# eric-downes/tianshou_marl

Hardware: AMD Instinct MI355X
Metric: env-steps/sec (n_env x n_agent) incl. PPO update, simple_spread N=3 (higher is better)
Workload: dtype f32; 1 GPU; simple_spread_v3 N=3 shared PPO, num_envs=1024 per GPU, obs 18, A=5, T=25, MLP 64-64; minibatch=4096, repeat=1, dispatch=per_agent, parallelism=env-shard x1

## Files before the change

include/tsmarl.h:

```cpp
#ifndef TSMARL_H
#define TSMARL_H

#include <stdint.h>

#ifdef __cplusplus
extern "C" {
#endif

#define TSM_ABI_VERSION 4

enum {
    TSM_OK = 0,
    TSM_ERR_INVALID = 1,
    TSM_ERR_HIP = 2,
    TSM_ERR_MALFORMED_BUFFER = 3,
    TSM_ERR_UNSUPPORTED = 4
};
#define TSM_VALUE

TSM_VALUE int tsm_abi_version(void);
const char *tsm_last_error(void);
int tsm_device_info(int *n_cu, int *wave_size, int64_t *hbm_bytes, char *name_out);

int tsm_kernel_option_get(const char *name, int32_t *value_out);
// ... 202 lines not shown
    tsm_mpe_cfg env;
    uint64_t env_seed;
    uint64_t *episode_ctr;
    float *agent_pos, *agent_vel, *landmark_pos;
    int32_t *steps;
    int32_t auto_reset, n_steps;
    float *obs_cur_out;
    void *vrb_state;
    int64_t sub_size;
    uint8_t *done_store;
    float *obs_store, *obs_next_store, *rew_store, *logp_store, *vs_store, *vnext_store;
    int32_t *act_store;
    uint8_t *term_store, *trunc_store;
    int64_t *ptr_out;
    double *ep_rew_out;
    int64_t *ep_len_out, *ep_idx_out;
    int64_t *ep_rec;
    int32_t max_ep, _pad2;
    uint64_t offset_inc;
    uint32_t *done_ctr;
} tsm_rollout_desc;

int tsm_rollout_spread(const tsm_rollout_desc *desc_host, void *stream);
int tsm_rollout_spread_actor(const tsm_rollout_desc *desc, void *stream);

typedef struct {
    int32_t n_env, n_adv, n_good, n_obst, max_cycles, _pad;
    double dt, damping, contact_force, contact_margin;
    double adv_size, good_size, obst_size;
    double adv_accel, good_accel, adv_speed, good_speed;
} tsm_mpe_tag_cfg;
TSM_VALUE int tsm_mpe_tag_obs_dim(const tsm_mpe_tag_cfg *cfg_host);
int tsm_mpe_tag_reset(const tsm_mpe_tag_cfg *cfg_host, uint64_t seed, uint64_t *episode_ctr,
                      const int64_t *env_ids, int64_t n_ids, float *agent_pos, float *agent_vel,
                      float *landmark_pos, int32_t *steps, float *obs_out, void *stream);
int tsm_mpe_tag_step(const tsm_mpe_tag_cfg *cfg_host, uint64_t seed, uint64_t *episode_ctr, const int32_t *act,
                     float *agent_pos, float *agent_vel, float *landmark_pos, int32_t *steps, float *obs_next_out,
                     float *obs_cur_out, float *rew_out, uint8_t *terminated_out, uint8_t *truncated_out,
                     uint8_t *done_env_out, int auto_reset, uint64_t *rng_tick, uint64_t rng_tick_inc, void *stream);
int tsm_u64_add(uint64_t *counter, uint64_t inc, void *stream);

typedef struct {
    const float *params[2];
    uint64_t policy_seed[2], offset[2];
    int32_t mode[2];
    int32_t obs_dim, hidden, n_act;
// ... 391 lines not shown
```

tianshou_marl_amd/algorithm/ppo.py:

```python
from __future__ import annotations

import os
import time
from typing import Literal

import numpy as np
import torch
from torch import nn

from .. import ops
from ..data.batch import Batch, split_bounds
from ..data.buffer import DeviceVectorReplayBuffer
from ..data.stats import (A2CTrainingStats, LazyDict, MapTrainingStats, ResultRing, lazy_training_stats, pinned_slot,
                          training_stats_from_steps)
from ..utils.net import DeviceRunningMeanStd, DiscreteActorCritic
from ..utils.tensor import to_tensor


class PPO(nn.Module):
    def __new__(cls, *args, **kw):
        if cls is PPO and kw.get("policy") is not None and kw.get("net") is None:
            from ..utils.net import MLPActorCritic, net_from_reference_modules

            if isinstance(net_from_reference_modules(kw["policy"], kw.get("critic"), kw.get("device", "cuda")), MLPActorCritic):
# ... 29 lines not shown
            lr, betas, adam_eps, weight_decay = kw_o["lr"], kw_o["betas"], kw_o["adam_eps"], kw_o["weight_decay"]
            sched_factory = getattr(optim, "lr_scheduler_factory", None)
        self._ctor = dict(lr=lr, betas=betas, adam_eps=adam_eps, weight_decay=weight_decay, eps_clip=eps_clip,
                          dual_clip=dual_clip, value_clip=value_clip, advantage_normalization=advantage_normalization,
                          recompute_advantage=recompute_advantage, vf_coef=vf_coef, ent_coef=ent_coef,
                          max_grad_norm=max_grad_norm, gae_lambda=gae_lambda, max_batchsize=max_batchsize, gamma=gamma,
                          return_scaling=return_scaling, deterministic_eval=deterministic_eval, dispatch=dispatch,
                          shuffle=shuffle, seed=seed, use_graph=use_graph, async_stats=async_stats)
        self._sched_factory = sched_factory
        self.net = net
        from ..env.spaces import Box, Discrete

        self.action_space = Discrete(net.n_act)
        self.observation_space = Box(-np.inf, np.inf, (net.obs_dim,))
        self._lr_dev = torch.tensor([float(lr)], dtype=torch.float64, device=net.flat.device)
        self._lr = float(lr)
        self.lr_schedulers: list = []
        if sched_factory is not None:
            self.lr_schedulers.append(sched_factory.create_scheduler(self))
        self.betas, self.adam_eps, self.weight_decay = betas, adam_eps, weight_decay
        self.eps_clip, self.dual_clip, self.value_clip = eps_clip, dual_clip, value_clip
        self.advantage_normalization, self.recompute_adv = advantage_normalization, recompute_advantage
        self.pack_rows = True
        self.vf_coef, self.ent_coef, self.max_grad_norm = vf_coef, ent_coef, max_grad_norm
        self.gae_lambda, self.gamma, self.max_batchsize = gae_lambda, gamma, max_batchsize
        self.return_scaling, self.ret_rms, self._eps = return_scaling, DeviceRunningMeanStd(net.flat.device), 1e-8
        self.deterministic_eval = deterministic_eval
        self.reuse_rollout_outputs = True
        self.is_within_training_step = False
        self.dispatch, self.shuffle = dispatch, shuffle
        self.use_graph = use_graph
        self.async_stats = async_stats
        self.seed = int(seed)
        dev = net.flat.device
        self.exp_avg = torch.zeros_like(net.flat.data)
        self.exp_avg_sq = torch.zeros_like(net.flat.data)
        self.opt_step = 0
        self._adam_work = torch.zeros(ops.call("tsm_adam_work_elems", net.flat.numel()), dtype=torch.float32, device=dev)
        self._sample_ctr = 0
        self._perm_ctr = torch.zeros(1, dtype=torch.int64, device=dev)
        self._cfg = ops.make_ppo_cfg(eps_clip, dual_clip, value_clip, advantage_normalization, vf_coef, ent_coef)
        self._ws: dict = {}
        self._grad_sync = None
        self.graph_collectives = os.environ.get("TSM_GRAPH_COLLECTIVES", "1") != "0"
        self.param_version = 0

# ... 26 lines not shown

    def forward(self, batch: Batch, state=None, **kwargs) -> Batch:
        obs = batch.obs
        if isinstance(obs, Batch) and "observations" in obs:
            from ..data.buffer import _obs_array

            obs = _obs_array(obs)
        elif isinstance(obs, Batch) and "obs" in obs:
            obs = obs.obs
        obs_t = torch.as_tensor(np.asarray(obs) if not isinstance(obs, torch.Tensor) else obs).to(self.device, torch.float32)
        lead = obs_t.shape[:-1]
        res = self.act_device(obs_t)
        return Batch(logits=res["logits"].reshape(*lead, -1), act=res["act"].reshape(lead).to(torch.int64),
                     state=None, policy=Batch(logp=res["logp"].reshape(lead), v_s=res["value"].reshape(lead)))

    def map_action(self, act):
        return act

    def map_action_inverse(self, act):
        return act

    def add_exploration_noise(self, act, batch):
        return act

    def _valid_rows(self, buffer: DeviceVectorReplayBuffer):
        lengths = buffer.index.lengths
        lens_h = lengths.cpu().numpy()
        S, B = buffer.sub_size, buffer.buffer_num
        uniform = bool((lens_h == lens_h[0]).all())
        ins_h = buffer.index.insertion_idx.cpu().numpy()
        start_h = (ins_h - lens_h) % S
        if uniform and (start_h == 0).all():
            T = int(lens_h[0])
            return T, None, None, None
        k = np.arange(S)[None, :]
        slot = (start_h[:, None] + k) % S
        valid = k < lens_h[:, None]
        rows = (slot * B + np.arange(B)[:, None])[valid]
        dev = self.device
        return S, torch.as_tensor(rows).to(dev), torch.as_tensor(start_h.astype(np.int32)).to(dev), \
            torch.as_tensor(lens_h.astype(np.int32)).to(dev)

    def _preprocess_batch(self, buffer: DeviceVectorReplayBuffer) -> dict:
        T, rows, env_start, env_len = self._valid_rows(buffer)
        B, N, D = buffer.buffer_num, buffer.n_agent, buffer.obs_dim
        L = B * N
# ... 309 lines not shown
            if self.advantage_normalization and not self.recompute_adv:
                seg = torch.arange(len(groups) * repeat, dtype=torch.int64, device=dev).view(-1, 1) * n_g
                w["mb_start_all"] = torch.cat([(seg + w["mb_start"][:-1].view(1, -1)).reshape(-1),
                                               torch.tensor([len(groups) * repeat * n_g], dtype=torch.int64, device=dev)])

            def preprocess(recompute: bool = False):
                if stored and not recompute:
                    if self.recompute_adv:
                        w["v_s"].copy_(buffer.vs_store[:T].reshape(T, L))
                        w["v_next"].copy_(buffer.vnext_store[:T].reshape(T, L))
                else:
                    img = self.net.image if recompute else None
                    ops.policy_forward(P, obs, A, H, mode="none" if recompute else "given", act=act,
                                       image=img,
                                       out=dict(value=w["v_s"].view(-1), logp=None if recompute else w["logp"],
                                                logits=None))
                    if no_next:
                        self._next_values_by_index(buffer, w["v_s"], T, None, out=w["v_next"])
                    else:
                        ops.policy_forward(P, obs_next, A, H, mode="none", image=img,
                                           out=dict(value=w["v_next"].view(-1), logits=None))
                self._gae(w["v_s"], w["v_next"], rew, term, trunc, N, out=(w["ret"], w["adv"]))

            def body():
                if self.shuffle == "device":
                    ops.random_permutations(n_g, len(groups) * repeat, self.seed ^ 0x5DEECE66D, counter_dev=w["step_dev"],
                                            scale=N if per_agent else 1, group_size=repeat,
                                            offset_mul=1 if per_agent else 0, out=w["perm"])
                preprocess()
                if "mb_start_all" in w and w["packed"] is not None:
                    ops.ppo_pack_minibatches(w["packed"], w["adv"], w["mb_start_all"], w["perm"].view(-1), obs, act, w["logp"],
                                             w["ret"].view(-1), w["v_s"].view(-1) if self.value_clip else None,
                                             out=w["stats"].view(-1, 2))
                    yield from self._global_adv_stats_steps(w["stats"].view(-1, 2), w["mb_start_all"])
                elif "mb_start_all" in w:
                    ops.ppo_adv_stats(w["adv"], w["mb_start_all"], perm=w["perm"].view(-1), out=w["stats"].view(-1, 2),
                                      max_rows=w["max_rows"])
                    yield from self._global_adv_stats_steps(w["stats"].view(-1, 2), w["mb_start_all"])
                pb = dict(obs=obs, act=act, logp_old=w["logp"], adv=w["adv"].view(-1), ret=w["ret"].view(-1),
                          v_s=w["v_s"].view(-1))
                k = 0
                for gi in range(len(groups)):
                    for r in range(repeat):
                        if self.recompute_adv and r > 0:
                            preprocess(recompute=True)
                        perm = w["perm"][gi, r]
                        if self.advantage_normalization and "mb_start_all" not in w:
                            ops.ppo_adv_stats(w["adv"], w["mb_start"], perm=perm, out=w["stats"][gi, r],
                                              max_rows=w["max_rows"])
                            yield from self._global_adv_stats_steps(w["stats"][gi, r], w["mb_start"])
                        for j, (s, e) in enumerate(bounds):
                            yield from self._grad_step_steps(
                                pb, perm[s:e], w["stats"][gi, r, j] if self.advantage_normalization else None, w["step_dev"],
                                plan=w, partial=w["partial"][k], image=self.net.image if k > 0 else None,
                                packed=None if w["packed"] is None else w["packed"]["rows"](k))
                            k += 1

            ops.capture_steps(w, body, self._sum_over_ranks, capture=self._capture_graph,
                              segmented=self._grad_sync is not None and not self.graph_collectives)
            if self.shuffle == "numpy":
                w["ref_ids"] = self._ref_ids(T, B, N, groups)
            self._ws[key] = g = w
        self._refill_host_perms(g)
        self._refill_step_dev(g)
        ops.replay_steps(g, self._sum_over_ranks)
        self._account_steps(g)
        slot = ResultRing.of(g, lambda: pinned_slot(*g["scal"].shape)).take(
            "expire" if self.async_stats else "resolve", "training stats were not read within 4 update() calls (async_stats=True)")
        ops.ppo_finalize_many(g["partial"], g["nb_max"] * 4, g["nb_dev"], g["M_dev"], self._cfg, slot["h"])
        sync = self._grad_sync
        if sync is not None:
            sync.post_check()
        slot["event"].record()

        out = lazy_training_stats(slot, sync, N if per_agent else None)
        if not self.async_stats:
            out.resolve()
        return out

    def update(self, buffer: DeviceVectorReplayBuffer, batch_size: int | None, repeat: int):
        if not self.is_within_training_step:
            raise RuntimeError(
                "update() was called outside of a training step as signalled by `is_within_training_step=False`; "
                "wrap the call in `policy_within_training_step(policy)` (tianshou/utils/torch_utils.py:31-46)")
        t0 = time.time()
        out = self._update(buffer, batch_size, repeat, t0)
        for sched in self.lr_schedulers:
            sched.step()
        out.train_time = time.time() - t0
# ... 331 lines not shown
```

tianshou_marl_amd/csrc/perm.hip:

```cpp
#include "common.h"
#include "philox.h"

namespace {

__device__ __forceinline__ uint32_t mix32(uint32_t x) {
    x ^= x >> 16; x *= 0x7feb352dU;
    x ^= x >> 15; x *= 0x846ca68bU;
    x ^= x >> 16;
    return x;
}

__device__ __forceinline__ void perm_point(int64_t n, int hb, uint64_t seed, uint64_t ctr, int64_t i, int p, int64_t scale,
                                           int32_t group_size, int64_t offset_mul, int64_t *__restrict__ out) {
    uint32_t k[4];
    tsm_philox4(seed, ctr + (uint64_t)p, k);
    const uint32_t mask = (1u << hb) - 1u;
    uint32_t x = (uint32_t)i;
    do {
        uint32_t l = x >> hb, r = x & mask;
#pragma unroll
        for (int round = 0; round < 6; ++round) {
            const uint32_t f = mix32(r + k[round & 3] + 0x9E3779B9u * (uint32_t)(round + 1)) & mask;
            const uint32_t t = l ^ f;
            l = r;
            r = t;
        }
        x = (l << hb) | r;
    } while ((int64_t)x >= n);
    out[(int64_t)p * n + i] = (int64_t)x * scale + (int64_t)(p / group_size) * offset_mul;
}

__global__ __launch_bounds__(256) void perm_kernel(int64_t n, int hb, uint64_t seed, uint64_t counter,
                                                    const uint64_t *__restrict__ counter_dev, int64_t scale,
                                                    int32_t group_size, int64_t offset_mul, int64_t *__restrict__ out) {
    const int64_t i = (int64_t)blockIdx.x * 256 + threadIdx.x;
    if (i >= n) return;
    perm_point(n, hb, seed, counter + (counter_dev ? *counter_dev : 0), i, blockIdx.y, scale, group_size, offset_mul, out);
}

__global__ __launch_bounds__(256) void perm_advance_kernel(int64_t n, int hb, uint64_t seed, uint64_t *counter_dev, uint64_t inc,
                                                            uint32_t *done_ctr, int64_t scale, int32_t group_size,
                                                            int64_t offset_mul, int64_t *__restrict__ out) {
    const uint64_t ctr = __hip_atomic_load(counter_dev, __ATOMIC_RELAXED, __HIP_MEMORY_SCOPE_AGENT);
    const int64_t i = (int64_t)blockIdx.x * 256 + threadIdx.x;
    if (i < n) perm_point(n, hb, seed, ctr, i, blockIdx.y, scale, group_size, offset_mul, out);
    __syncthreads();
    if (threadIdx.x == 0 && atomicAdd(done_ctr, 1u) == gridDim.x * gridDim.y - 1) {
        __hip_atomic_store(counter_dev, ctr + inc, __ATOMIC_RELAXED, __HIP_MEMORY_SCOPE_AGENT);
        *done_ctr = 0u;
    }
}

}

TSM_EXPORT int tsm_random_permutations(int64_t n, int32_t n_perm, uint64_t seed, uint64_t counter,
                                       const uint64_t *counter_dev, int64_t scale, int32_t group_size,
                                       int64_t offset_mul, int64_t *out, void *stream) {
    TSM_REQUIRE(n >= 0 && n < ((int64_t)1 << 30), "tsm_random_permutations: n=%lld out of range [0, 2^30)", (long long)n);
    TSM_REQUIRE(n_perm >= 0 && n_perm <= 65535, "tsm_random_permutations: n_perm out of range");
    TSM_REQUIRE(group_size >= 1, "tsm_random_permutations: group_size must be >= 1");
    if (n == 0 || n_perm == 0) return TSM_OK;
    TSM_REQUIRE(out, "tsm_random_permutations: null output");
    int bits = 0;
    while (((int64_t)1 << bits) < n) ++bits;
    const int hb = bits < 2 ? 1 : (bits + 1) / 2;
    hipLaunchKernelGGL(perm_kernel, dim3((unsigned)ceil_div(n, 256), (unsigned)n_perm), dim3(256), 0, tsm_stream(stream),
                       n, hb, seed, counter, counter_dev, scale, group_size, offset_mul, out);
    TSM_LAUNCH_CHECK();
    return TSM_OK;
}

TSM_EXPORT int tsm_random_permutations_advance(int64_t n, int32_t n_perm, uint64_t seed, uint64_t *counter_dev, uint64_t counter_inc,
                                               uint32_t *done_ctr, int64_t scale, int32_t group_size, int64_t offset_mul,
                                               int64_t *out, void *stream) {
    TSM_REQUIRE(n >= 1 && n < ((int64_t)1 << 30), "tsm_random_permutations_advance: n=%lld out of range [1, 2^30)", (long long)n);
    TSM_REQUIRE(n_perm >= 1 && n_perm <= 65535, "tsm_random_permutations_advance: n_perm out of range");
    TSM_REQUIRE(group_size >= 1, "tsm_random_permutations_advance: group_size must be >= 1");
    TSM_REQUIRE(out && counter_dev && done_ctr, "tsm_random_permutations_advance: null pointer");
    int bits = 0;
    while (((int64_t)1 << bits) < n) ++bits;
    const int hb = bits < 2 ? 1 : (bits + 1) / 2;
    hipLaunchKernelGGL(perm_advance_kernel, dim3((unsigned)ceil_div(n, 256), (unsigned)n_perm), dim3(256), 0, tsm_stream(stream),
                       n, hb, seed, counter_dev, counter_inc, done_ctr, scale, group_size, offset_mul, out);
    TSM_LAUNCH_CHECK();
    return TSM_OK;
}
```

tianshou_marl_amd/csrc/rollout.hip:

```cpp
#include "common.h"
#include "mlp_tile.h"
#include "mpe_dev.h"
#include "philox.h"
#include "rollout_dev.h"
#include "rollout_fwd.h"
#include "wave_mlp.h"

int tsm_mpe_check_cfg(const tsm_mpe_cfg *h, MpeCfg *c);
extern long long *g_tsm_stamps;

namespace {

struct RolloutArgs {
    const float *P, *img;
    Dims d;
    uint64_t pol_seed, offset;
    const uint64_t *offset_dev;
    int mode;
    MpeCfg c;
    uint64_t env_seed;
    uint64_t *episode_ctr;
    float *apos, *avel, *lpos;
    int32_t *steps;
    int auto_reset;
    float *obs_cur_out;
    RolloutBufArgs b;
    long long *stamps;
};


#define XSTAMP(k) do { if (a.stamps && blockIdx.x == 0 && threadIdx.x == 0 && t < 4) a.stamps[900 + t * 8 + (k)] = (long long)wall_clock64(); } while (0)
#define STAMP(k) do { if (a.stamps && blockIdx.x == 0 && threadIdx.x == 0 && t < 4) a.stamps[t * 8 + (k)] = (long long)wall_clock64(); } while (0)

struct RtLay {
    int XN0, AP, AV, LP, REW, LOGP, VAL, MIN, ACT, STEPS, DONE, ROW, EP, CX, CY, CV, U, ANY, total;
    __host__ __device__ RtLay(int fwd_total, int ld1) {
        int o = fwd_total;
        XN0 = o; o += R * ld1;
        AP = o; o += R * 2;
        AV = o; o += R * 2;
        LP = o; o += R * 2;
        REW = o; o += R;
        LOGP = o; o += R;
        VAL = o; o += R;
        MIN = o; o += R;
        ACT = o; o += R;
        STEPS = o; o += R;
        DONE = o; o += 2 * R;
        o = (o + 1) & ~1;
        ROW = o; o += 2 * 2 * R;
        EP = o; o += 2 * R;
        o = (o + 3) & ~3;
        CX = o; o += R * 8;
        CY = o; o += R * 8;
        CV = o; o += R * 8;
        U = o; o += 2 * R;
        ANY = o; o += 2;
        o += 3 * R + 12;
        total = o;
    }
};

template <int H, int NT2, int DS = 0, int NS = 0>
__global__ __launch_bounds__(NT2) void rollout_kernel(RolloutArgs a) {
    extern __shared__ __attribute__((aligned(16))) float lds[];
    const Dims d = DS ? dims_const(DS, 5) : a.d;
    MpeCfg c_ = a.c;
    if (NS) { c_.N = NS; c_.obs_dim = DS; }
    const MpeCfg c = c_;
    const Lay<H> ly(d, false);
    const int N = c.N, D = d.D, st = 2 * N;
    const int EPB = R / N;
    const int e0 = blockIdx.x * EPB;
    const int n_here = min(EPB, c.n_env - e0);
    const int rows_here = n_here * N;
    const int64_t B = c.n_env;
    const RtLay tl(ly.total, d.ld1);
    float *XN0 = lds + tl.XN0, *s_ap = lds + tl.AP, *s_av = lds + tl.AV, *s_lp = lds + tl.LP, *s_rew = lds + tl.REW,
          *s_logp = lds + tl.LOGP, *s_val = lds + tl.VAL, *s_m = lds + tl.MIN, *s_cx = lds + tl.CX, *s_cy = lds + tl.CY, *s_u = lds + tl.U;
    int *s_act = reinterpret_cast<int *>(lds + tl.ACT), *s_steps = reinterpret_cast<int *>(lds + tl.STEPS),
        *s_done = reinterpret_cast<int *>(lds + tl.DONE), *s_cv = reinterpret_cast<int *>(lds + tl.CV),
        *s_any = reinterpret_cast<int *>(lds + tl.ANY);
    int64_t *s_row = reinterpret_cast<int64_t *>(lds + tl.ROW);
    uint64_t *s_ep = reinterpret_cast<uint64_t *>(lds + tl.EP);

    if (a.stamps && threadIdx.x == 0 && blockIdx.x < 256) a.stamps[64 + 2 * blockIdx.x] = (long long)wall_clock64();
    const bool main_t = threadIdx.x < NT;
    if (main_t) {
// ... 255 lines not shown
                    const int rr = i / D, k = i - rr * D, ee = rr / N;
                    if (s_done[g + ee])
                        XN[rr * d.ld1 + k] =
                            mpe_obs_elem(c, s_ap + ee * st, s_av + ee * st, s_lp + ee * st, rr - ee * N, k);
                }
                __syncthreads();
            }
        }
        { const int tmp = xcur; xcur = xnxt; xnxt = tmp; }
        STAMP(6);
    }
    __syncthreads();
    if (a.stamps && threadIdx.x == 0 && blockIdx.x < 256) a.stamps[65 + 2 * blockIdx.x] = (long long)wall_clock64();
    for (int i = threadIdx.x; i < n_here * st; i += NT2) {
        a.apos[(int64_t)e0 * st + i] = s_ap[i];
        a.avel[(int64_t)e0 * st + i] = s_av[i];
        a.lpos[(int64_t)e0 * st + i] = s_lp[i];
    }
    if (env_lane) {
        a.steps[be] = s_steps[bel];
        vl.store(vs, a.b.ep_rec, be);
    }
    if (ret_lane) epr.store(vs, N, e0 + rq);
    rollout_advance_counter(a.b.done_ctr, a.b.offset_dev_rw, a.b.offset_inc, threadIdx.x == 0);
}

struct Rw64Lay {
    static constexpr int kLdc = 68;
    int AP, AV, LP, LG, H2C, VAL, CX, CY, CV, MIN, REW, LOGP, ACT, STEPS, DONE, ROW, EP, size;
    __host__ __device__ Rw64Lay() {
        int q = 0;
        AP = q; q += 2 * R;
        AV = q; q += 2 * R;
        LP = q; q += 2 * R;
        LG = q; q += R * 16;
        H2C = q; q += R * kLdc;
        VAL = q; q += R;
        CX = q; q += R * 8;
        CY = q; q += R * 8;
        CV = q; q += R * 8;
        MIN = q; q += R;
        REW = q; q += R;
        LOGP = q; q += R;
        ACT = q; q += R;
        STEPS = q; q += R;
        DONE = q; q += R;
        ROW = q; q += 2 * R;
// ... 248 lines not shown
        a.apos[(int64_t)e0 * st + lane] = s_ap[lane];
        a.avel[(int64_t)e0 * st + lane] = s_av[lane];
        a.lpos[(int64_t)e0 * st + lane] = s_lp[lane];
    }
    if (env_lane) {
        a.steps[be] = s_steps[bel];
        vl.store(vs, a.b.ep_rec, be);
        epr.store(vs, N, be);
    }
    rollout_advance_counter(a.b.done_ctr, a.b.offset_dev_rw, a.b.offset_inc, tid == 0);
}

__global__ void u64_add_kernel(uint64_t *p, uint64_t inc) { *p += inc; }

}

TSM_EXPORT int tsm_u64_add(uint64_t *counter, uint64_t inc, void *stream) {
    TSM_REQUIRE(counter, "tsm_u64_add: null pointer");
    hipLaunchKernelGGL(u64_add_kernel, dim3(1), dim3(1), 0, tsm_stream(stream), counter, inc);
    TSM_LAUNCH_CHECK();
    return TSM_OK;
}

TSM_EXPORT int tsm_rollout_spread(const tsm_rollout_desc *desc_host, void *stream) {
    TSM_REQUIRE(desc_host, "tsm_rollout_spread: null descriptor");
    const tsm_rollout_desc &h = *desc_host;
    RolloutArgs a;
    if (int rc = make_dims(h.obs_dim, h.hidden, h.n_act, &a.d)) return rc;
    if (int rc = tsm_mpe_check_cfg(&h.env, &a.c)) return rc;
    TSM_REQUIRE(a.c.obs_dim == h.obs_dim, "tsm_rollout_spread: obs_dim %d != 6 * n_agent", h.obs_dim);
    TSM_REQUIRE(h.n_act == 5, "tsm_rollout_spread: simple_spread has 5 discrete actions");
    TSM_REQUIRE(a.c.N <= R, "tsm_rollout_spread: n_agent exceeds the row tile");
    TSM_REQUIRE(h.n_steps >= 1 && h.sub_size >= 1, "tsm_rollout_spread: bad n_steps / sub_size");
    TSM_REQUIRE(h.mode == 1 || h.mode == 2, "tsm_rollout_spread: mode must be 1 (sample) or 2 (argmax)");
    TSM_REQUIRE((h.params || h.param_image) && h.episode_ctr && h.agent_pos && h.agent_vel && h.landmark_pos && h.steps,
                "tsm_rollout_spread: null pointer");
    if (int rc = rollout_buf_args(h, "tsm_rollout_spread", &a.b)) return rc;
    a.P = h.params; a.img = h.param_image;
    a.pol_seed = h.policy_seed; a.offset = h.offset; a.offset_dev = h.offset_dev; a.mode = h.mode;
    a.env_seed = h.env_seed; a.episode_ctr = h.episode_ctr;
    a.apos = h.agent_pos; a.avel = h.agent_vel; a.lpos = h.landmark_pos; a.steps = h.steps;
    a.auto_reset = h.auto_reset; a.obs_cur_out = h.obs_cur_out;
    a.stamps = g_tsm_stamps;
    const Lay<64> ly(a.d, false);
    {
        const int form = tsm_opt(TSM_OPT_ROLLOUT_FORM);
        const int64_t total_waves = ceil_div(a.c.n_env, R / a.c.N);
        if (a.d.nJ <= 3 && (form == 2 || (form == 0 && total_waves > 256))) {
            int n_waves = 1;
            while (n_waves < 4 && ceil_div(total_waves, n_waves) > 256) n_waves *= 2;
// ... 20 lines not shown
            } else
            switch (a.d.nJ) {
                case 1: LAUNCHW(1); break;
                case 2: LAUNCHW(2); break;
                default: LAUNCHW(3); break;
            }
#undef LAUNCHW
            TSM_LAUNCH_CHECK();
            return TSM_OK;
        }
    }
    const size_t shmem = (size_t)RtLay(ly.total, a.d.ld1).total * sizeof(float);
    static bool attr_set = false;
    if (!attr_set) {
        TSM_HIP(tsm_allow_max_lds(reinterpret_cast<const void *>(rollout_kernel<64, NT>)));
        TSM_HIP(tsm_allow_max_lds(reinterpret_cast<const void *>(rollout_kernel<64, 2 * NT>)));
        TSM_HIP(tsm_allow_max_lds(reinterpret_cast<const void *>(rollout_kernel<64, 2 * NT, 18, 3>)));
        attr_set = true;
    }
    const int EPB = R / a.c.N;
    const unsigned n_wg = (unsigned)ceil_div(a.c.n_env, EPB);
    const bool eight = n_wg <= 256 || shmem > 80 * 1024;
    const bool c18 = a.d.D == 18 && a.d.A == 5 && a.c.N == 3 && !tsm_opt(TSM_OPT_GENERIC);
    if (eight && c18) hipLaunchKernelGGL((rollout_kernel<64, 2 * NT, 18, 3>), dim3(n_wg), dim3(2 * NT), shmem, tsm_stream(stream), a);
    else if (eight) hipLaunchKernelGGL((rollout_kernel<64, 2 * NT>), dim3(n_wg), dim3(2 * NT), shmem, tsm_stream(stream), a);
    else hipLaunchKernelGGL((rollout_kernel<64, NT>), dim3(n_wg), dim3(NT), shmem, tsm_stream(stream), a);
    TSM_LAUNCH_CHECK();
    return TSM_OK;
}
```

tianshou_marl_amd/csrc/rollout_dev.h:

```cpp
#pragma once
#include "common.h"
#include "vrb_dev.h"

struct RolloutBufArgs {
    void *vrb_state;
    int64_t S;
    uint8_t *done_store;
    float *obs_store, *obs_next_store, *rew_store, *logp_store, *vs_store, *vnext_store;
    int32_t *act_store;
    uint8_t *term_store, *trunc_store;
    int64_t *ptr_out, *ep_len_out, *ep_idx_out;
    double *ep_rew_out;
    int n_steps;
    int64_t *ep_rec;
    int max_ep;
    uint64_t offset_inc;
    uint64_t *offset_dev_rw;
    uint32_t *done_ctr;
};

template <class Desc>
int rollout_buf_args(const Desc &h, const char *entry, RolloutBufArgs *b) {
    TSM_REQUIRE(h.vrb_state && h.done_store && h.obs_store && h.act_store && h.rew_store && h.term_store && h.trunc_store &&
                    h.ptr_out && h.ep_rew_out && h.ep_len_out && h.ep_idx_out,
// ... 25 lines not shown
        for (int k = 0; k < MAXN; ++k) if (k < N) acc[k] = vs.ep_return[be * N + k];
    }
    __device__ __forceinline__ void fold(double *ep_rew_out, int64_t *ep_rec, int max_ep, int N, int64_t B, int64_t be, int64_t o, bool tr,
                                         bool rec, int &n_fin, const float *rew) {
        double *rec_rew = rec ? reinterpret_cast<double *>(ep_rec + B + (int64_t)B * max_ep) +
                                    ((int64_t)be * max_ep + n_fin) * N : nullptr;
#pragma unroll
        for (int k = 0; k < MAXN; ++k) {
            if (k < N) {
                const double ac = acc[k] + (double)rew[k];
                ep_rew_out[o * N + k] = tr ? ac : 0.0;
                if (rec) rec_rew[k] = ac;
                acc[k] = tr ? 0.0 : ac;
            }
        }
        n_fin += tr ? 1 : 0;
    }
    __device__ __forceinline__ void store(const VrbState &vs, int N, int64_t be) const {
#pragma unroll
        for (int k = 0; k < MAXN; ++k) if (k < N) vs.ep_return[be * N + k] = acc[k];
    }
};

__device__ __forceinline__ void rollout_advance_counter(uint32_t *done_ctr, uint64_t *offset_dev_rw, uint64_t offset_inc, bool first) {
    if (done_ctr && first) {
        if (atomicAdd(done_ctr, 1u) == gridDim.x - 1) {
            *offset_dev_rw += offset_inc;
            *done_ctr = 0u;
        }
    }
}
```

tianshou_marl_amd/data/collector.py:

```python
from __future__ import annotations

import time
import warnings
from copy import copy
from typing import Any, Callable

import numpy as np
import torch

from .. import ops
from .batch import Batch
from .buffer import DeviceVectorReplayBuffer
from .stats import CollectStats, ResultRing


_EXPIRED = ("these CollectStats were not read within 4 collect() calls and their pinned staging buffer was recycled "
            "(Collector(async_stats=True)); read them earlier or use async_stats=False")


class LazyCollectStats(CollectStats):

    _LAZY = ("returns", "lens", "n_collected_episodes", "returns_stat", "lens_stat")

    def __init__(self, collector: "Collector", slot: dict, steps: int) -> None:
# ... 38 lines not shown
                self.__dict__[k] = getattr(full, k)
            self._col.collect_episode += self.__dict__["n_collected_episodes"]
            object.__setattr__(self, "_done", True)
            if slot["pending"] is self:
                slot["pending"] = None
        return self

    def __getattribute__(self, name):
        if name in LazyCollectStats._LAZY and not object.__getattribute__(self, "_done"):
            object.__getattribute__(self, "resolve")()
        return object.__getattribute__(self, name)


class Collector:
    def __init__(self, policy, env, buffer: DeviceVectorReplayBuffer | None = None, exploration_noise: bool = False,
                 on_episode_done_hook: Callable | None = None, on_step_hook: Callable | None = None,
                 raise_on_nan_in_buffer: bool = False, collect_stats_class: type = CollectStats, use_graph: bool = True,
                 fused_rollout: bool = True, async_stats: bool = False) -> None:
        self.use_graph = use_graph
        self.async_stats = async_stats
        self.collect_stats_class = collect_stats_class
        self.fused_rollout = fused_rollout
        self.stage_episode_record = False
        self.policy = getattr(policy, "policy", policy)
        self.env = env
        self.env_num = len(env)
        if buffer is None:
            raise ValueError("a DeviceVectorReplayBuffer is required (the buffer lives in HBM)")
        if hasattr(buffer, "bind") and not buffer.allocated and hasattr(env, "n_agent") and hasattr(env, "obs_dim"):
            buffer.bind(env.n_agent, env.obs_dim)
        if buffer.buffer_num < self.env_num:
            raise ValueError(f"Buffer has only {buffer.buffer_num} sub-buffers for {self.env_num} envs")
        self.buffer = buffer
        self.exploration_noise = exploration_noise
        self.on_episode_done_hook, self.on_step_hook = on_episode_done_hook, on_step_hook
        self.raise_on_nan_in_buffer = raise_on_nan_in_buffer
        self.collect_step = self.collect_episode = 0
        self.collect_time = 0.0
        self._pre_obs = None
        self._pre_info = None
        self._pred_std: list = []
        self._device_path = hasattr(env, "step_device") and hasattr(self.policy, "act_device")
        self._ws: dict = {}
        if self._device_path:
            from ..utils.host import warn_if_oversubscribed

# ... 231 lines not shown
    def _rollout_fused(self, n_iter: int, ws: dict, deterministic: bool, rec_host=None) -> None:
        import ctypes as C

        from .._abi import call, ptr, stream_ptr, tsm_rollout_desc

        env, buf, pol = self.env, self.buffer, self._single_policy()
        if hasattr(env, "_tag_cfg"):
            return self._rollout_fused_tag(n_iter, ws, rec_host)
        actor_only = self._can_fuse_actor()
        actor = self._actor_of(pol) if actor_only else None
        entry = "tsm_rollout_spread_actor" if actor_only else "tsm_rollout_spread"

        def mark():
            if actor_only:
                buf.policy_outputs_version = None
                buf.behaviour_outputs_version = None
                buf.column_outputs = None
                buf.mark_logp_outputs(getattr(pol, "param_version", None))
            else:
                buf.mark_policy_outputs(getattr(pol, "param_version", -1))
                buf.mark_column_outputs([(id(pol), getattr(pol, "param_version", None))] * buf.n_agent)
            buf.note_uniform_rows(n_iter)

        img = getattr(getattr(pol, "net", None), "image", None)
        flat = actor.flat.data if actor_only else pol.net.flat.data
        ctr0 = int(getattr(pol, "_sample_ctr", 0))
        dkey = ("desc", n_iter, deterministic, env._pp, pol.seed, ctr0, env._seed, int(env.auto_reset), buf.storage_key(),
                flat.data_ptr(), 0 if img is None else img.data_ptr(), env.agent_pos.data_ptr())
        if dkey in self._ws:
            d = self._ws[dkey]
            d.ep_rec = rec_host.data_ptr() if rec_host is not None else None
            call(entry, C.byref(d), stream_ptr())
            mark()
            return
        d = tsm_rollout_desc()
        self._ws[dkey] = d
        d.params, d.param_image = ptr(flat), None
        d.obs_dim, d.hidden, d.n_act, d.mode = env.obs_dim, (128 if actor_only else pol.net.hidden), env.n_act, 2 if deterministic else 1
        d.policy_seed, d.offset, d.offset_dev = pol.seed & (2**64 - 1), ctr0, ptr(env.rng_tick)
        d.env, d.env_seed, d.episode_ctr = env._cfg, env._seed & (2**64 - 1), ptr(env.episode_ctr)
        d.agent_pos, d.agent_vel, d.landmark_pos = ptr(env.agent_pos), ptr(env.agent_vel), ptr(env.landmark_pos)
        d.steps, d.auto_reset, d.n_steps = ptr(env.steps), int(env.auto_reset), n_iter
        d.obs_cur_out = ptr(env.obs_cur)
        d.vrb_state, d.sub_size, d.done_store = ptr(buf.index.state), buf.sub_size, ptr(buf.done_store)
        d.obs_store, d.obs_next_store, d.rew_store = ptr(buf.obs_store), ptr(buf.obs_next_store), ptr(buf.rew_store)
        d.logp_store, d.vs_store, d.vnext_store = ptr(buf.logp_store), ptr(buf.vs_store), ptr(buf.vnext_store)
        d.act_store, d.term_store, d.trunc_store = ptr(buf.act_store), ptr(buf.term_store), ptr(buf.trunc_store)
        d.ptr_out, d.ep_rew_out = ptr(ws["ptr"]), ptr(ws["ep_rew"])
        d.ep_len_out, d.ep_idx_out = ptr(ws["ep_len"]), ptr(ws["ep_idx"])
        if rec_host is not None:
            d.ep_rec, d.max_ep = rec_host.data_ptr(), ws["max_ep"]
        if "done_ctr" not in ws:
            ws["done_ctr"] = torch.zeros(1, dtype=torch.int32, device=buf.device)
        d.offset_inc, d.done_ctr = n_iter * self.env_num * buf.n_agent, ptr(ws["done_ctr"])
        call(entry, C.byref(d), stream_ptr())
        mark()

    def _rollout_fused_tag(self, n_iter: int, ws: dict, rec_host=None) -> None:
        import ctypes as C

        from .._abi import call, ptr, stream_ptr, tsm_rollout_tag_desc

        env, buf = self.env, self.buffer
        teams = self._tag_teams()
        modes = tuple(2 if (getattr(p, "deterministic_eval", False) and not getattr(p, "is_within_training_step", False))
                      else 1 for p in teams)
        dkey = ("tag_desc", n_iter, modes, env._pp, tuple(p.seed for p in teams), tuple(p._sample_ctr for p in teams),
                env._seed, int(env.auto_reset), buf.storage_key(), tuple(p.net.flat.data_ptr() for p in teams),
                env.agent_pos.data_ptr())
        d = self._ws.get(dkey)
        if d is None:
            d = tsm_rollout_tag_desc()
            self._ws[dkey] = d
            for k, p in enumerate(teams):
                d.params[k], d.policy_seed[k], d.offset[k] = ptr(p.net.flat.data), p.seed & (2**64 - 1), p._sample_ctr
                d.mode[k] = modes[k]
            d.obs_dim, d.hidden, d.n_act, d.offset_dev = env.obs_dim, 64, env.n_act, ptr(env.rng_tick)
            d.env_major_counter = int(teams[0] is teams[1])
# ... 241 lines not shown
```

Measured before the change: 171.6 million env-steps/s.

## Generate PPO minibatch permutations in idle workgroups of the rollout kernel

Adds extra workgroups to the fused spread rollout launch. When the grid is smaller than the CU count, these fill the next PPO update's device permutation buffer on otherwise idle CUs. The PPO update then replays a separately captured graph that skips the permutation kernel, saving one launch and its serial time. In exchange it adds handshake state between collector and policy, a second captured graph, and a completion counter that must now count only rollout tiles. It also depends on the step counter being unchanged between rollout and update.

```diff
diff --git a/include/tsmarl.h b/include/tsmarl.h
--- a/include/tsmarl.h
+++ b/include/tsmarl.h
@@ -248,6 +248,10 @@
 } tsm_rollout_desc;
 
 int tsm_rollout_spread(const tsm_rollout_desc *desc_host, void *stream);
+int tsm_rollout_spread_prep(const tsm_rollout_desc *desc_host, int64_t perm_n, int32_t n_perm, uint64_t perm_seed,
+                            const uint64_t *perm_counter_dev, int64_t perm_scale, int32_t perm_group_size,
+                            int64_t perm_offset_mul, int64_t *perm_out, int32_t n_cu, int32_t *taken_out, void *stream);
+int tsm_rollout_prep_extra(int64_t tiles, int32_t n_cu, int64_t perm_n, int32_t n_perm, int32_t *extra_out);
 int tsm_rollout_spread_actor(const tsm_rollout_desc *desc, void *stream);
 
 typedef struct {
diff --git a/tianshou_marl_amd/algorithm/ppo.py b/tianshou_marl_amd/algorithm/ppo.py
--- a/tianshou_marl_amd/algorithm/ppo.py
+++ b/tianshou_marl_amd/algorithm/ppo.py
@@ -75,6 +75,10 @@
         self.eps_clip, self.dual_clip, self.value_clip = eps_clip, dual_clip, value_clip
         self.advantage_normalization, self.recompute_adv = advantage_normalization, recompute_advantage
         self.pack_rows = True
+        self.rollout_prep = True
+        self._prep_offer = None
+        self._prep_gen = 0
+        self._prep_filled = None
         self.vf_coef, self.ent_coef, self.max_grad_norm = vf_coef, ent_coef, max_grad_norm
         self.gae_lambda, self.gamma, self.max_batchsize = gae_lambda, gamma, max_batchsize
         self.return_scaling, self.ret_rms, self._eps = return_scaling, DeviceRunningMeanStd(net.flat.device), 1e-8
@@ -147,6 +151,19 @@
 
     def add_exploration_noise(self, act, batch):
         return act
+
+    def rollout_prep_request(self, buffer: DeviceVectorReplayBuffer) -> dict | None:
+        self._prep_filled = None
+        if not (self.rollout_prep and self.is_within_training_step and self._prep_offer is not None):
+            return None
+        key, g = self._prep_offer
+        if self._ws.get(key) is not g or key[1] != buffer.storage_key() or g.get("step_host") != self.opt_step:
+            return None
+        self._prep_gen += 1
+        return dict(g["perm_request"], gen=self._prep_gen, key=key)
+
+    def rollout_prep_done(self, req: dict, taken: bool) -> None:
+        self._prep_filled = (req["gen"], req["key"], self.opt_step) if taken else None
 
     def _valid_rows(self, buffer: DeviceVectorReplayBuffer):
         lengths = buffer.index.lengths
@@ -502,8 +519,10 @@
                                            out=dict(value=w["v_next"].view(-1), logits=None))
                 self._gae(w["v_s"], w["v_next"], rew, term, trunc, N, out=(w["ret"], w["adv"]))
 
+            skip_perm = [False]
+
             def body():
-                if self.shuffle == "device":
+                if self.shuffle == "device" and not skip_perm[0]:
                     ops.random_permutations(n_g, len(groups) * repeat, self.seed ^ 0x5DEECE66D, counter_dev=w["step_dev"],
                                             scale=N if per_agent else 1, group_size=repeat,
                                             offset_mul=1 if per_agent else 0, out=w["perm"])
@@ -540,11 +559,35 @@
                               segmented=self._grad_sync is not None and not self.graph_collectives)
             if self.shuffle == "numpy":
                 w["ref_ids"] = self._ref_ids(T, B, N, groups)
+            if (self.shuffle == "device" and self._grad_sync is None and not self.recompute_adv
+                    and self.advantage_normalization and w["packed"] is not None):
+                w["perm_request"] = dict(out=w["perm"], n=n_g, n_perm=len(groups) * repeat, seed=self.seed ^ 0x5DEECE66D,
+                                         counter_dev=w["step_dev"], scale=N if per_agent else 1, group_size=repeat,
+                                         offset_mul=1 if per_agent else 0)
+
+                def capture_prepared():
+                    w2: dict = {}
+                    skip_perm[0] = True
+                    try:
+                        ops.capture_steps(w2, body, self._sum_over_ranks, capture=self._capture_graph)
+                    finally:
+                        skip_perm[0] = False
+                    w["graph_prep"] = w2["graph"]
+
+                w["capture_prepared"] = capture_prepared
             self._ws[key] = g = w
         self._refill_host_perms(g)
-        self._refill_step_dev(g)
-        ops.replay_steps(g, self._sum_over_ranks)
+        filled, self._prep_filled = self._prep_filled, None
+        if (self.rollout_prep and "perm_request" in g and g.get("step_host") == self.opt_step
+                and filled == (self._prep_gen, key, self.opt_step)):
+            if g.get("graph_prep") is None:
+                g["capture_prepared"]()
+            g["graph_prep"].replay()
+        else:
+            self._refill_step_dev(g)
+            ops.replay_steps(g, self._sum_over_ranks)
         self._account_steps(g)
+        self._prep_offer = (key, g) if self.rollout_prep and "perm_request" in g else None
         slot = ResultRing.of(g, lambda: pinned_slot(*g["scal"].shape)).take(
             "expire" if self.async_stats else "resolve", "training stats were not read within 4 update() calls (async_stats=True)")
         ops.ppo_finalize_many(g["partial"], g["nb_max"] * 4, g["nb_dev"], g["M_dev"], self._cfg, slot["h"])
diff --git a/tianshou_marl_amd/csrc/perm.hip b/tianshou_marl_amd/csrc/perm.hip
--- a/tianshou_marl_amd/csrc/perm.hip
+++ b/tianshou_marl_amd/csrc/perm.hip
@@ -1,34 +1,8 @@
 #include "common.h"
+#include "perm_dev.h"
 #include "philox.h"
 
 namespace {
-
-__device__ __forceinline__ uint32_t mix32(uint32_t x) {
-    x ^= x >> 16; x *= 0x7feb352dU;
-    x ^= x >> 15; x *= 0x846ca68bU;
-    x ^= x >> 16;
-    return x;
-}
-
-__device__ __forceinline__ void perm_point(int64_t n, int hb, uint64_t seed, uint64_t ctr, int64_t i, int p, int64_t scale,
-                                           int32_t group_size, int64_t offset_mul, int64_t *__restrict__ out) {
-    uint32_t k[4];
-    tsm_philox4(seed, ctr + (uint64_t)p, k);
-    const uint32_t mask = (1u << hb) - 1u;
-    uint32_t x = (uint32_t)i;
-    do {
-        uint32_t l = x >> hb, r = x & mask;
-#pragma unroll
-        for (int round = 0; round < 6; ++round) {
-            const uint32_t f = mix32(r + k[round & 3] + 0x9E3779B9u * (uint32_t)(round + 1)) & mask;
-            const uint32_t t = l ^ f;
-            l = r;
-            r = t;
-        }
-        x = (l << hb) | r;
-    } while ((int64_t)x >= n);
-    out[(int64_t)p * n + i] = (int64_t)x * scale + (int64_t)(p / group_size) * offset_mul;
-}
 
 __global__ __launch_bounds__(256) void perm_kernel(int64_t n, int hb, uint64_t seed, uint64_t counter,
                                                     const uint64_t *__restrict__ counter_dev, int64_t scale,
@@ -61,9 +35,7 @@
     TSM_REQUIRE(group_size >= 1, "tsm_random_permutations: group_size must be >= 1");
     if (n == 0 || n_perm == 0) return TSM_OK;
     TSM_REQUIRE(out, "tsm_random_permutations: null output");
-    int bits = 0;
-    while (((int64_t)1 << bits) < n) ++bits;
-    const int hb = bits < 2 ? 1 : (bits + 1) / 2;
+    const int hb = perm_half_bits(n);
     hipLaunchKernelGGL(perm_kernel, dim3((unsigned)ceil_div(n, 256), (unsigned)n_perm), dim3(256), 0, tsm_stream(stream),
                        n, hb, seed, counter, counter_dev, scale, group_size, offset_mul, out);
     TSM_LAUNCH_CHECK();
@@ -77,9 +49,7 @@
     TSM_REQUIRE(n_perm >= 1 && n_perm <= 65535, "tsm_random_permutations_advance: n_perm out of range");
     TSM_REQUIRE(group_size >= 1, "tsm_random_permutations_advance: group_size must be >= 1");
     TSM_REQUIRE(out && counter_dev && done_ctr, "tsm_random_permutations_advance: null pointer");
-    int bits = 0;
-    while (((int64_t)1 << bits) < n) ++bits;
-    const int hb = bits < 2 ? 1 : (bits + 1) / 2;
+    const int hb = perm_half_bits(n);
     hipLaunchKernelGGL(perm_advance_kernel, dim3((unsigned)ceil_div(n, 256), (unsigned)n_perm), dim3(256), 0, tsm_stream(stream),
                        n, hb, seed, counter_dev, counter_inc, done_ctr, scale, group_size, offset_mul, out);
     TSM_LAUNCH_CHECK();
diff --git a/tianshou_marl_amd/csrc/perm_dev.h b/tianshou_marl_amd/csrc/perm_dev.h
--- /dev/null
+++ b/tianshou_marl_amd/csrc/perm_dev.h
@@ -0,0 +1,53 @@
+#pragma once
+#include "common.h"
+#include "philox.h"
+
+static inline int perm_half_bits(int64_t n) {
+    int bits = 0;
+    while (((int64_t)1 << bits) < n) ++bits;
+    return bits < 2 ? 1 : (bits + 1) / 2;
+}
+
+__device__ __forceinline__ uint32_t perm_mix32(uint32_t x) {
+    x ^= x >> 16; x *= 0x7feb352dU;
+    x ^= x >> 15; x *= 0x846ca68bU;
+    x ^= x >> 16;
+    return x;
+}
+
+__device__ __forceinline__ void perm_point(int64_t n, int hb, uint64_t seed, uint64_t ctr, int64_t i, int p, int64_t scale,
+                                           int32_t group_size, int64_t offset_mul, int64_t *__restrict__ out) {
+    uint32_t k[4];
+    tsm_philox4(seed, ctr + (uint64_t)p, k);
+    const uint32_t mask = (1u << hb) - 1u;
+    uint32_t x = (uint32_t)i;
+    do {
+        uint32_t l = x >> hb, r = x & mask;
+#pragma unroll
+        for (int round = 0; round < 6; ++round) {
+            const uint32_t f = perm_mix32(r + k[round & 3] + 0x9E3779B9u * (uint32_t)(round + 1)) & mask;
+            const uint32_t t = l ^ f;
+            l = r;
+            r = t;
+        }
+        x = (l << hb) | r;
+    } while ((int64_t)x >= n);
+    out[(int64_t)p * n + i] = (int64_t)x * scale + (int64_t)(p / group_size) * offset_mul;
+}
+
+struct PermReq {
+    int64_t *out;
+    const uint64_t *counter_dev;
+    int64_t n, scale, offset_mul;
+    uint64_t seed;
+    int32_t n_perm, group_size, hb;
+};
+
+__device__ __forceinline__ void perm_fill(const PermReq &q, int wg, int n_wg) {
+    const uint64_t ctr = __hip_atomic_load(q.counter_dev, __ATOMIC_RELAXED, __HIP_MEMORY_SCOPE_AGENT);
+    const int64_t total = q.n * q.n_perm, stride = (int64_t)n_wg * blockDim.x;
+    for (int64_t j = (int64_t)wg * blockDim.x + threadIdx.x; j < total; j += stride) {
+        const int p = (int)(j / q.n);
+        perm_point(q.n, q.hb, q.seed, ctr, j - (int64_t)p * q.n, p, q.scale, q.group_size, q.offset_mul, q.out);
+    }
+}
diff --git a/tianshou_marl_amd/csrc/rollout.hip b/tianshou_marl_amd/csrc/rollout.hip
--- a/tianshou_marl_amd/csrc/rollout.hip
+++ b/tianshou_marl_amd/csrc/rollout.hip
@@ -1,6 +1,9 @@
+#include <algorithm>
+
 #include "common.h"
 #include "mlp_tile.h"
 #include "mpe_dev.h"
+#include "perm_dev.h"
 #include "philox.h"
 #include "rollout_dev.h"
 #include "rollout_fwd.h"
@@ -26,6 +29,8 @@
     float *obs_cur_out;
     RolloutBufArgs b;
     long long *stamps;
+    int tiles;
+    PermReq perm;
 };
 
 
@@ -61,9 +66,15 @@
     }
 };
 
-template <int H, int NT2, int DS = 0, int NS = 0>
+template <int H, int NT2, int DS = 0, int NS = 0, bool PERM = false>
 __global__ __launch_bounds__(NT2) void rollout_kernel(RolloutArgs a) {
     extern __shared__ __attribute__((aligned(16))) float lds[];
+    if constexpr (PERM) {
+        if ((int)blockIdx.x >= a.tiles) {
+            perm_fill(a.perm, (int)blockIdx.x - a.tiles, (int)gridDim.x - a.tiles);
+            return;
+        }
+    }
     const Dims d = DS ? dims_const(DS, 5) : a.d;
     MpeCfg c_ = a.c;
     if (NS) { c_.N = NS; c_.obs_dim = DS; }
@@ -365,7 +376,8 @@
         vl.store(vs, a.b.ep_rec, be);
     }
     if (ret_lane) epr.store(vs, N, e0 + rq);
-    rollout_advance_counter(a.b.done_ctr, a.b.offset_dev_rw, a.b.offset_inc, threadIdx.x == 0);
+    if constexpr (PERM) rollout_advance_counter(a.b.done_ctr, a.b.offset_dev_rw, a.b.offset_inc, threadIdx.x == 0, (unsigned)a.tiles);
+    else rollout_advance_counter(a.b.done_ctr, a.b.offset_dev_rw, a.b.offset_inc, threadIdx.x == 0);
 }
 
 struct Rw64Lay {
@@ -660,10 +672,18 @@
     return TSM_OK;
 }
 
-TSM_EXPORT int tsm_rollout_spread(const tsm_rollout_desc *desc_host, void *stream) {
+static int rollout_prep_extra(int64_t tiles, int n_cu, int64_t entries) {
+    if (entries <= 0 || tiles >= n_cu) return 0;
+    const int64_t idle = n_cu - tiles, useful = ceil_div(entries, (int64_t)(2 * NT));
+    return (int)std::min<int64_t>(std::min<int64_t>(idle, useful), 64);
+}
+
+static int rollout_spread_launch(const tsm_rollout_desc *desc_host, const PermReq *prep, int n_cu, int32_t *taken, void *stream) {
     TSM_REQUIRE(desc_host, "tsm_rollout_spread: null descriptor");
     const tsm_rollout_desc &h = *desc_host;
     RolloutArgs a;
+    a.tiles = 0;
+    a.perm = PermReq{};
     if (int rc = make_dims(h.obs_dim, h.hidden, h.n_act, &a.d)) return rc;
     if (int rc = tsm_mpe_check_cfg(&h.env, &a.c)) return rc;
     TSM_REQUIRE(a.c.obs_dim == h.obs_dim, "tsm_rollout_spread: obs_dim %d != 6 * n_agent", h.obs_dim);
@@ -730,9 +750,62 @@
     const unsigned n_wg = (unsigned)ceil_div(a.c.n_env, EPB);
     const bool eight = n_wg <= 256 || shmem > 80 * 1024;
     const bool c18 = a.d.D == 18 && a.d.A == 5 && a.c.N == 3 && !tsm_opt(TSM_OPT_GENERIC);
+    const int extra = prep && eight ? rollout_prep_extra(n_wg, n_cu, prep->n * prep->n_perm) : 0;
+    if (extra > 0) {
+        static bool attr_prep = false;
+        if (!attr_prep) {
+            TSM_HIP(tsm_allow_max_lds(reinterpret_cast<const void *>(rollout_kernel<64, 2 * NT, 0, 0, true>)));
+            TSM_HIP(tsm_allow_max_lds(reinterpret_cast<const void *>(rollout_kernel<64, 2 * NT, 18, 3, true>)));
+            attr_prep = true;
+        }
+        a.tiles = (int)n_wg;
+        a.perm = *prep;
+        if (c18) hipLaunchKernelGGL((rollout_kernel<64, 2 * NT, 18, 3, true>), dim3(n_wg + extra), dim3(2 * NT), shmem, tsm_stream(stream), a);
+        else hipLaunchKernelGGL((rollout_kernel<64, 2 * NT, 0, 0, true>), dim3(n_wg + extra), dim3(2 * NT), shmem, tsm_stream(stream), a);
+        TSM_LAUNCH_CHECK();
+        if (taken) *taken = 1;
+        return TSM_OK;
+    }
     if (eight && c18) hipLaunchKernelGGL((rollout_kernel<64, 2 * NT, 18, 3>), dim3(n_wg), dim3(2 * NT), shmem, tsm_stream(stream), a);
     else if (eight) hipLaunchKernelGGL((rollout_kernel<64, 2 * NT>), dim3(n_wg), dim3(2 * NT), shmem, tsm_stream(stream), a);
     else hipLaunchKernelGGL((rollout_kernel<64, NT>), dim3(n_wg), dim3(NT), shmem, tsm_stream(stream), a);
     TSM_LAUNCH_CHECK();
     return TSM_OK;
 }
+
+TSM_EXPORT int tsm_rollout_spread(const tsm_rollout_desc *desc_host, void *stream) {
+    return rollout_spread_launch(desc_host, nullptr, 0, nullptr, stream);
+}
+
+TSM_EXPORT int tsm_rollout_prep_extra(int64_t tiles, int32_t n_cu, int64_t perm_n, int32_t n_perm, int32_t *extra_out) {
+    TSM_REQUIRE(extra_out, "tsm_rollout_prep_extra: null output");
+    TSM_REQUIRE(tiles >= 0 && n_cu >= 0 && perm_n >= 0 && n_perm >= 0, "tsm_rollout_prep_extra: negative argument");
+    *extra_out = rollout_prep_extra(tiles, n_cu, perm_n * n_perm);
+    return TSM_OK;
+}
+
+TSM_EXPORT int tsm_rollout_spread_prep(const tsm_rollout_desc *desc_host, int64_t perm_n, int32_t n_perm, uint64_t perm_seed,
+                                       const uint64_t *perm_counter_dev, int64_t perm_scale, int32_t perm_group_size,
+                                       int64_t perm_offset_mul, int64_t *perm_out, int32_t n_cu, int32_t *taken_out, void *stream) {
+    TSM_REQUIRE(taken_out, "tsm_rollout_spread_prep: null taken_out");
+    *taken_out = 0;
+    if (!perm_out || perm_n == 0 || n_perm == 0) return rollout_spread_launch(desc_host, nullptr, 0, nullptr, stream);
+    TSM_REQUIRE(perm_n > 0 && perm_n < ((int64_t)1 << 30), "tsm_rollout_spread_prep: perm_n=%lld out of range [0, 2^30)", (long long)perm_n);
+    TSM_REQUIRE(n_perm > 0 && n_perm <= 65535, "tsm_rollout_spread_prep: n_perm out of range");
+    TSM_REQUIRE(perm_group_size >= 1, "tsm_rollout_spread_prep: perm_group_size must be >= 1");
+    TSM_REQUIRE(perm_counter_dev, "tsm_rollout_spread_prep: the permutation request needs its device counter");
+    TSM_REQUIRE(n_cu >= 0, "tsm_rollout_spread_prep: negative n_cu");
+    if (n_cu == 0) {
+        static int dev_cu = 0;
+        if (!dev_cu) {
+            int dev = 0;
+            TSM_HIP(hipGetDevice(&dev));
+            TSM_HIP(hipDeviceGetAttribute(&dev_cu, hipDeviceAttributeMultiprocessorCount, dev));
+        }
+        n_cu = dev_cu;
+    }
+    PermReq q;
+    q.out = perm_out; q.counter_dev = perm_counter_dev; q.n = perm_n; q.scale = perm_scale; q.offset_mul = perm_offset_mul;
+    q.seed = perm_seed; q.n_perm = n_perm; q.group_size = perm_group_size; q.hb = perm_half_bits(perm_n);
+    return rollout_spread_launch(desc_host, &q, n_cu, taken_out, stream);
+}
diff --git a/tianshou_marl_amd/csrc/rollout_dev.h b/tianshou_marl_amd/csrc/rollout_dev.h
--- a/tianshou_marl_amd/csrc/rollout_dev.h
+++ b/tianshou_marl_amd/csrc/rollout_dev.h
@@ -71,11 +71,15 @@
     }
 };
 
-__device__ __forceinline__ void rollout_advance_counter(uint32_t *done_ctr, uint64_t *offset_dev_rw, uint64_t offset_inc, bool first) {
+__device__ __forceinline__ void rollout_advance_counter(uint32_t *done_ctr, uint64_t *offset_dev_rw, uint64_t offset_inc, bool first,
+                                                        unsigned n_wg) {
     if (done_ctr && first) {
-        if (atomicAdd(done_ctr, 1u) == gridDim.x - 1) {
+        if (atomicAdd(done_ctr, 1u) == n_wg - 1) {
             *offset_dev_rw += offset_inc;
             *done_ctr = 0u;
         }
     }
 }
+__device__ __forceinline__ void rollout_advance_counter(uint32_t *done_ctr, uint64_t *offset_dev_rw, uint64_t offset_inc, bool first) {
+    rollout_advance_counter(done_ctr, offset_dev_rw, offset_inc, first, gridDim.x);
+}
diff --git a/tianshou_marl_amd/data/collector.py b/tianshou_marl_amd/data/collector.py
--- a/tianshou_marl_amd/data/collector.py
+++ b/tianshou_marl_amd/data/collector.py
@@ -84,6 +84,7 @@
         self.collect_stats_class = collect_stats_class
         self.fused_rollout = fused_rollout
         self.stage_episode_record = False
+        self.prep_n_cu = 0
         self.policy = getattr(policy, "policy", policy)
         self.env = env
         self.env_num = len(env)
@@ -361,6 +362,18 @@
                 buf.mark_column_outputs([(id(pol), getattr(pol, "param_version", None))] * buf.n_agent)
             buf.note_uniform_rows(n_iter)
 
+        def launch(d):
+            ask = None if actor_only else getattr(pol, "rollout_prep_request", None)
+            req = ask(buf) if ask is not None else None
+            if req is None:
+                call(entry, C.byref(d), stream_ptr())
+                return
+            taken = C.c_int32(0)
+            call("tsm_rollout_spread_prep", C.byref(d), req["n"], req["n_perm"], req["seed"] & (2**64 - 1), ptr(req["counter_dev"]),
+                 req["scale"], req["group_size"], req["offset_mul"], ptr(req["out"]), int(self.prep_n_cu), C.byref(taken),
+                 stream_ptr())
+            pol.rollout_prep_done(req, bool(taken.value))
+
         img = getattr(getattr(pol, "net", None), "image", None)
         flat = actor.flat.data if actor_only else pol.net.flat.data
         ctr0 = int(getattr(pol, "_sample_ctr", 0))
@@ -369,7 +382,7 @@
         if dkey in self._ws:
             d = self._ws[dkey]
             d.ep_rec = rec_host.data_ptr() if rec_host is not None else None
-            call(entry, C.byref(d), stream_ptr())
+            launch(d)
             mark()
             return
         d = tsm_rollout_desc()
@@ -392,7 +405,7 @@
         if "done_ctr" not in ws:
             ws["done_ctr"] = torch.zeros(1, dtype=torch.int32, device=buf.device)
         d.offset_inc, d.done_ctr = n_iter * self.env_num * buf.n_agent, ptr(ws["done_ctr"])
-        call(entry, C.byref(d), stream_ptr())
+        launch(d)
         mark()
 
     def _rollout_fused_tag(self, n_iter: int, ws: dict, rec_host=None) -> None:
```

After: 173.4 million env-steps/s (median of 6 runs). +1.1%, better.
